# lly00412/MF-NeRF

Measured on AMD Instinct MI355X. Metric: training rays/sec + test PSNR, Synthetic-NeRF Lego 30k steps, higher is better.
Workload: dtype f16-mfma/f32; 1 GPU; Lego 800x800 training step, 8192 rays/batch/GPU, Hash L16 F2 T2^19, rgb 64x2; preset=lego, global_batch=8192, parallelism=dp1

## Files before the change

### mf-nerf_amd/csrc/vren_composite.hip

```cpp
#include "composite_sample.hpp"
#include "wave_ops.hpp"
#include "vren_launch.hpp"

using namespace mfn;
using namespace mfn_vren;

namespace {


__device__ __forceinline__ float t_chain(float a, float& T_run, float thr, int lane, int n_valid, int* stop) {
    constexpr int WAVE_SHR1 = 0x138;
    const float b = 1.0f - a;
    const float bs = __int_as_float(
        __builtin_amdgcn_update_dpp(__float_as_int(1.0f), __float_as_int(b), WAVE_SHR1, 0xF, 0xF, false));
    const int t0 = __float_as_int(T_run);
    float X = T_run;
    const int nv = __builtin_amdgcn_readfirstlane(n_valid);
    for (int k = 1; k < nv; ++k)
        X = __int_as_float(__builtin_amdgcn_update_dpp(t0, __float_as_int(X), WAVE_SHR1, 0xF, 0xF, false)) * bs;
    const float Ta = X * b;
    const uint64_t hit = __ballot(lane < n_valid && Ta <= thr);
    const int st = hit ? (int)__builtin_ctzll(hit) : 64;
    T_run = readlane_f(Ta, st < 64 ? st : n_valid - 1);
    *stop = st;
    return X;
}

__global__ __launch_bounds__(256) void composite_fw_wave_kernel(
    const float* __restrict__ sigmas, const float* __restrict__ rgbs, const float* __restrict__ deltas,
    const float* __restrict__ ts, const int64_t* __restrict__ rays_a, int64_t n_rays, float T_thr,
    int64_t* __restrict__ total_samples, float* __restrict__ opacity, float* __restrict__ depth,
    float* __restrict__ rgb, float* __restrict__ ws) {
    const int lane = threadIdx.x & 63;
    const int64_t n = ((int64_t)blockIdx.x * blockDim.x + threadIdx.x) >> 6;
    if (n >= n_rays) return;
    const int64_t ray = rays_a[3 * n], start = rays_a[3 * n + 1];
    const int N = (int)rays_a[3 * n + 2];
    float T = 1.0f, R = 0.f, G = 0.f, B = 0.f, D = 0.f, O = 0.f;
    int total = N;
    bool ended = false;
    for (int k0 = 0; k0 < N; k0 += 64) {
        const int nv = min(64, N - k0);
        const int64_t s = start + k0 + lane;
        const bool valid = lane < nv;
        float w = 0.0f;
        if (!ended) {
            const float a = valid ? 1.0f - fast_exp(-sigmas[s] * deltas[s]) : 0.0f;
            int stop;
            const float myT = t_chain(a, T, T_thr, lane, nv, &stop);
            if (valid && lane <= stop) {
                w = a * myT;
                R = fmaf(w, rgbs[3 * s], R); G = fmaf(w, rgbs[3 * s + 1], G); B = fmaf(w, rgbs[3 * s + 2], B);
                D = fmaf(w, ts[s], D);
                O += w;
            }
            if (stop < 64) { ended = true; total = k0 + stop; }
        }
        if (valid) ws[s] = w;
    }
    R = wave_sum(R); G = wave_sum(G); B = wave_sum(B); D = wave_sum(D); O = wave_sum(O);
    if (lane == 0) {
        opacity[ray] = O; depth[ray] = D;
        rgb[3 * ray] = R; rgb[3 * ray + 1] = G; rgb[3 * ray + 2] = B;
        total_samples[ray] = total;
    }
}

__global__ __launch_bounds__(256) void composite_bw_wave_kernel(
    const float* __restrict__ dL_dopacity, const float* __restrict__ dL_ddepth, const float* __restrict__ dL_drgb,
    const float* __restrict__ dL_dws, const float* __restrict__ sigmas, const float* __restrict__ rgbs,
    const float* __restrict__ ws, const float* __restrict__ deltas, const float* __restrict__ ts,
    const int64_t* __restrict__ rays_a, const float* __restrict__ opacity, const float* __restrict__ depth,
    const float* __restrict__ rgb, int64_t n_rays, float T_thr, float* __restrict__ dL_dsigmas,
    float* __restrict__ dL_drgbs) {
    const int lane = threadIdx.x & 63;
    const int64_t n = ((int64_t)blockIdx.x * blockDim.x + threadIdx.x) >> 6;
    if (n >= n_rays) return;
    const int64_t ray = rays_a[3 * n], start = rays_a[3 * n + 1];
    const int N = (int)rays_a[3 * n + 2];
    if (N <= 0) return;
    float wsum = 0.0f;
    for (int k0 = 0; k0 < N; k0 += 64) {
        const int64_t s = start + k0 + lane;
        if (k0 + lane < N) wsum += dL_dws[s] * ws[s];
    }
    wsum = wave_sum(wsum);
    const float Rt = rgb[3 * ray], Gt = rgb[3 * ray + 1], Bt = rgb[3 * ray + 2];
    const float O = opacity[ray], Dt = depth[ray];
    const float gr = dL_drgb[3 * ray], gg = dL_drgb[3 * ray + 1], gb = dL_drgb[3 * ray + 2];
    const float go = dL_dopacity[ray], gd = dL_ddepth[ray];
    float T = 1.0f, cr = 0.f, cg = 0.f, cb = 0.f, cd = 0.f, cs = 0.f;
    bool ended = false;
    for (int k0 = 0; k0 < N; k0 += 64) {
        const int nv = min(64, N - k0);
        const int64_t s = start + k0 + lane;
        const bool valid = lane < nv;
        float dsig = 0.0f, d0 = 0.0f, d1 = 0.0f, d2 = 0.0f;
        if (!ended) {
            float sg = 0.f, dl = 0.f, c0 = 0.f, c1 = 0.f, c2 = 0.f, tv = 0.f, dw = 0.f, wv = 0.f;
            if (valid) {
                sg = sigmas[s]; dl = deltas[s]; tv = ts[s]; dw = dL_dws[s]; wv = ws[s];
                c0 = rgbs[3 * s]; c1 = rgbs[3 * s + 1]; c2 = rgbs[3 * s + 2];
            }
            const float a = valid ? 1.0f - fast_exp(-sg * dl) : 0.0f;
            int stop;
            const float myT = t_chain(a, T, T_thr, lane, nv, &stop);
            const bool act = valid && lane <= stop;
            const float w = act ? a * myT : 0.0f;
            const float Tn = myT * (1.0f - a);
            const float pr = wave_incl_scan(w * c0) + cr, pg = wave_incl_scan(w * c1) + cg;
            const float pb = wave_incl_scan(w * c2) + cb, pd = wave_incl_scan(w * tv) + cd;
            const float ps = wave_incl_scan(act ? dw * wv : 0.0f) + cs;
            cr = readlane_f(pr, 63); cg = readlane_f(pg, 63); cb = readlane_f(pb, 63); cd = readlane_f(pd, 63);
            cs = readlane_f(ps, 63);
            if (act) {
                d0 = gr * w; d1 = gg * w; d2 = gb * w;
                float acc = gr * fmaf(c0, Tn, -(Rt - pr));
                acc = fmaf(gg, fmaf(c1, Tn, -(Gt - pg)), acc);
                acc = fmaf(gb, fmaf(c2, Tn, -(Bt - pb)), acc);
                acc = fmaf(go, 1 - O, acc);
                acc = fmaf(gd, fmaf(tv, Tn, -(Dt - pd)), acc);
                acc = fmaf(Tn, dw, acc);
                acc = acc - (wsum - ps);
                dsig = dl * acc;
            }
            if (stop < 64) ended = true;
        }
        if (valid) {
            dL_dsigmas[s] = dsig;
            dL_drgbs[3 * s] = d0; dL_drgbs[3 * s + 1] = d1; dL_drgbs[3 * s + 2] = d2;
        }
    }
}

struct BgUnused {};
template <bool DEV_BG> struct BgParam { using first = float; using rest = float; };
template <> struct BgParam<true> { using first = const float*; using rest = BgUnused; };
template <bool DEV_BG>
__device__ __forceinline__ void bg_fetch(typename BgParam<DEV_BG>::first a0, typename BgParam<DEV_BG>::rest a1,
                                         typename BgParam<DEV_BG>::rest a2, float& b0, float& b1, float& b2) {
    if constexpr (DEV_BG) { b0 = a0[0]; b1 = a0[1]; b2 = a0[2]; }
    else { b0 = a0; b1 = a1; b2 = a2; }
}

template <bool DEV_BG>
__global__ __launch_bounds__(256) void composite_fused_wave_kernel(
    const float* __restrict__ sigmas, const float* __restrict__ rgbs, const float* __restrict__ deltas,
    const float* __restrict__ ts, const int64_t* __restrict__ rays_a, int64_t n_rays, float T_thr,
    const float* __restrict__ target, int64_t n_mean, float lambda_o, typename BgParam<DEV_BG>::first bg0,
    typename BgParam<DEV_BG>::rest bg1, typename BgParam<DEV_BG>::rest bg2,
    int64_t* __restrict__ total_samples, float* __restrict__ opacity, float* __restrict__ depth,
    float* __restrict__ rgb, float* __restrict__ ws, float* __restrict__ dL_drgb, float* __restrict__ dL_dop,
    float* __restrict__ dL_dsigmas, float* __restrict__ dL_drgbs, float* __restrict__ loss_part) {
    __shared__ float lsum[4];
    const int lane = threadIdx.x & 63, wid = threadIdx.x >> 6;
    const int64_t n = ((int64_t)blockIdx.x * blockDim.x + threadIdx.x) >> 6;
    float l = 0.0f;
    if (n < n_rays) {
        const int64_t ray = rays_a[3 * n], start = rays_a[3 * n + 1];
        const int N = (int)rays_a[3 * n + 2];
        const float tg[3] = {target[3 * ray], target[3 * ray + 1], target[3 * ray + 2]};
        float b0, b1, b2;
        bg_fetch<DEV_BG>(bg0, bg1, bg2, b0, b1, b2);
        float T = 1.0f, R = 0.f, G = 0.f, B = 0.f, D = 0.f, O = 0.f;
        int total = N;
        bool ended = false;
        for (int k0 = 0; k0 < N; k0 += 64) {
            const int nv = min(64, N - k0);
            const int64_t s = start + k0 + lane;
            const bool valid = lane < nv;
            float w = 0.0f, tn = 0.0f;
            if (!ended) {
                float sg = 0.f, dl = 0.f, c0 = 0.f, c1 = 0.f, c2 = 0.f, tv = 0.f;
                if (valid) {
                    sg = sigmas[s]; dl = deltas[s]; tv = ts[s];
                    c0 = rgbs[3 * s]; c1 = rgbs[3 * s + 1]; c2 = rgbs[3 * s + 2];
                }
                const float a = valid ? 1.0f - fast_exp(-sg * dl) : 0.0f;
                int stop;
                const float myT = t_chain(a, T, T_thr, lane, nv, &stop);
                if (valid && lane <= stop) {
                    w = a * myT;
                    tn = myT * (1.0f - a);
                    R = fmaf(w, c0, R); G = fmaf(w, c1, G); B = fmaf(w, c2, B);
                    D = fmaf(w, tv, D);
                    O += w;
                }
                if (stop < 64) { ended = true; total = k0 + stop; }
            }
            if (valid) { ws[s] = w; dL_dsigmas[s] = tn; }
        }
        R = wave_sum(R); G = wave_sum(G); B = wave_sum(B); D = wave_sum(D); O = wave_sum(O);
        const float inv3n = 1.0f / (3.0f * (float)n_mean), invn = 1.0f / (float)n_mean;
        const float bg[3] = {b0, b1, b2}, col[3] = {R, G, B};
        float gcol[3], dop = 0.0f;
#pragma unroll
        for (int c = 0; c < 3; ++c) {
            const float e = col[c] + bg[c] * (1.0f - O) - tg[c];
            l += e * e * inv3n;
            gcol[c] = 2.0f * e * inv3n;
            dop -= bg[c] * gcol[c];
        }
        const float o = O + 1e-10f;
        l += lambda_o * (-o * logf(o)) * invn;
        const float go = dop + lambda_o * (-(logf(o) + 1.0f)) * invn;
        if (lane == 0) {
            opacity[ray] = O; depth[ray] = D;
            rgb[3 * ray] = R; rgb[3 * ray + 1] = G; rgb[3 * ray + 2] = B;
            total_samples[ray] = total;
            dL_drgb[3 * ray] = gcol[0]; dL_drgb[3 * ray + 1] = gcol[1]; dL_drgb[3 * ray + 2] = gcol[2];
            dL_dop[ray] = go;
        }
        const int last = ended ? total : N - 1;
        const float gr = gcol[0], gg = gcol[1], gb = gcol[2];
        float cr = 0.f, cg = 0.f, cb = 0.f;
        for (int k0 = 0; k0 < N; k0 += 64) {
            const int64_t s = start + k0 + lane;
            const bool valid = k0 + lane < N;
            const bool act = k0 + lane <= last;
            if (k0 > last) {
                if (valid) {
                    dL_dsigmas[s] = 0.0f;
                    dL_drgbs[3 * s] = 0.0f; dL_drgbs[3 * s + 1] = 0.0f; dL_drgbs[3 * s + 2] = 0.0f;
                }
                continue;
            }
            float w = 0.f, tn = 0.f, c0 = 0.f, c1 = 0.f, c2 = 0.f, dl = 0.f;
            if (act) {
                w = ws[s]; tn = dL_dsigmas[s]; dl = deltas[s];
                c0 = rgbs[3 * s]; c1 = rgbs[3 * s + 1]; c2 = rgbs[3 * s + 2];
            }
            const float pr = wave_incl_scan(w * c0) + cr, pg = wave_incl_scan(w * c1) + cg;
            const float pb = wave_incl_scan(w * c2) + cb;
            cr = readlane_f(pr, 63); cg = readlane_f(pg, 63); cb = readlane_f(pb, 63);
            float dsig = 0.0f, d0 = 0.0f, d1 = 0.0f, d2 = 0.0f;
            if (act) {
                d0 = gr * w; d1 = gg * w; d2 = gb * w;
                float acc = gr * fmaf(c0, tn, -(R - pr));
                acc = fmaf(gg, fmaf(c1, tn, -(G - pg)), acc);
                acc = fmaf(gb, fmaf(c2, tn, -(B - pb)), acc);
                acc = fmaf(go, 1 - O, acc);
                dsig = dl * acc;
            }
            if (valid) {
                dL_dsigmas[s] = dsig;
                dL_drgbs[3 * s] = d0; dL_drgbs[3 * s + 1] = d1; dL_drgbs[3 * s + 2] = d2;
            }
        }
    }
    if (lane == 0) lsum[wid] = l;
    __syncthreads();
    if (threadIdx.x == 0 && loss_part) loss_part[blockIdx.x] = (lsum[0] + lsum[1]) + (lsum[2] + lsum[3]);
}

__global__ void composite_test_kernel(const float* __restrict__ sigmas, const float* __restrict__ rgbs,
                                      const float* __restrict__ deltas, const float* __restrict__ ts,
                                      int64_t* __restrict__ alive, int64_t n_alive, int N_samples, float T_thr,
                                      const int32_t* __restrict__ n_eff, float* __restrict__ opacity,
                                      float* __restrict__ depth, float* __restrict__ rgb) {
    const int64_t n = (int64_t)blockIdx.x * blockDim.x + threadIdx.x;
    if (n >= n_alive) return;
    const int ne = n_eff[n];
    if (ne == 0) { alive[n] = -1; return; }
    const int64_t r = alive[n];
    RaySums S;
    S.O = opacity[r]; S.D = depth[r]; S.R = rgb[3 * r]; S.G = rgb[3 * r + 1]; S.B = rgb[3 * r + 2];
    S.T = 1 - S.O;
    for (int s = 0; s < ne; ++s) {
        const int64_t k = n * N_samples + s;
        const float sg = sigmas[k], dl = deltas[k];
        const float c0 = rgbs[3 * k], c1 = rgbs[3 * k + 1], c2 = rgbs[3 * k + 2];
        const float tv = ts[k];
        if (composite_sample(S, sg, dl, tv, c0, c1, c2, T_thr)) { alive[n] = -1; break; }
    }
    opacity[r] = S.O; depth[r] = S.D; rgb[3 * r] = S.R; rgb[3 * r + 1] = S.G; rgb[3 * r + 2] = S.B;
}

__global__ void distortion_fw_kernel(const float* __restrict__ ws, const float* __restrict__ deltas,
                                     const float* __restrict__ ts, const int64_t* __restrict__ rays_a,
                                     int64_t n_rays, float* __restrict__ loss, float* __restrict__ ws_incl,
                                     float* __restrict__ wts_incl) {
    const int64_t n = (int64_t)blockIdx.x * blockDim.x + threadIdx.x;
    if (n >= n_rays) return;
    const int64_t ray = rays_a[3 * n], start = rays_a[3 * n + 1];
    const int N = (int)rays_a[3 * n + 2];
    const float third = 1.0f / 3;
    float a = 0.f, b = 0.f, sum = 0.f;
    for (int k = 0; k < N; ++k) {
        const int64_t s = start + k;
        const float wx = a, wtx = b;
        a += ws[s]; b += ws[s] * ts[s];
        ws_incl[s] = a; wts_incl[s] = b;
        sum += 2 * (b * wx - a * wtx) + third * ws[s] * ws[s] * deltas[s];
    }
    loss[ray] = sum;
}

__global__ void distortion_bw_kernel(const float* __restrict__ dL_dloss, const float* __restrict__ ws_incl,
                                     const float* __restrict__ wts_incl, const float* __restrict__ ws,
                                     const float* __restrict__ deltas, const float* __restrict__ ts,
                                     const int64_t* __restrict__ rays_a, int64_t n_rays, float* __restrict__ dL_dws) {
    const int64_t n = (int64_t)blockIdx.x * blockDim.x + threadIdx.x;
    if (n >= n_rays) return;
    const int64_t ray = rays_a[3 * n], start = rays_a[3 * n + 1];
    const int N = (int)rays_a[3 * n + 2];
    if (N <= 0) return;
    const int64_t end = start + N - 1;
    const float ws_sum = ws_incl[end], wts_sum = wts_incl[end], g = dL_dloss[ray];
    for (int64_t s = start; s <= end; ++s) {
        const float first = (s == start) ? 0.0f : fmaf(ts[s], ws_incl[s - 1], -wts_incl[s - 1]);
        const float second = fmaf(-ts[s], ws_sum - ws_incl[s], wts_sum - wts_incl[s]);
        float v = g * 2 * (first + second);
        dL_dws[s] = fmaf(g * (float)2 / 3 * ws[s], deltas[s], v);
    }
}


template <bool DEV_BG>
__global__ void nerf_loss_kernel(const float* __restrict__ rgb, const float* __restrict__ opacity,
                                 const float* __restrict__ gt, int64_t n_rays, int64_t n_mean, float lambda_o,
                                 typename BgParam<DEV_BG>::first bg0, typename BgParam<DEV_BG>::rest bg1,
                                 typename BgParam<DEV_BG>::rest bg2, float* __restrict__ dL_drgb,
                                 float* __restrict__ dL_dop, float* __restrict__ loss_sum) {
    const int64_t r = (int64_t)blockIdx.x * blockDim.x + threadIdx.x;
    float l = 0.0f;
    if (r < n_rays) {
        const float op = opacity[r];
        const float inv3n = 1.0f / (3.0f * (float)n_mean), invn = 1.0f / (float)n_mean;
        float b0, b1, b2;
        bg_fetch<DEV_BG>(bg0, bg1, bg2, b0, b1, b2);
        const float bg[3] = {b0, b1, b2};
        float dop = 0.0f;
#pragma unroll
        for (int c = 0; c < 3; ++c) {
            const float e = rgb[3 * r + c] + bg[c] * (1.0f - op) - gt[3 * r + c];
            l += e * e * inv3n;
            const float g = 2.0f * e * inv3n;
            dL_drgb[3 * r + c] = g;
            dop -= bg[c] * g;
        }
        const float o = op + 1e-10f;
        l += lambda_o * (-o * logf(o)) * invn;
        dL_dop[r] = dop + lambda_o * (-(logf(o) + 1.0f)) * invn;
    }
    for (int off = 32; off > 0; off >>= 1) l += __shfl_down(l, off, 64);
    if ((threadIdx.x & 63) == 0 && loss_sum) atomicAdd(loss_sum, l);
}

template <bool DEV_BG>
int composite_train_fused_launch(const char* what, const float* sigmas, const float* rgbs, const float* deltas,
                                 const float* ts, const int64_t* rays_a, int64_t n_rays, int64_t n_samples,
                                 float T_threshold, const float* target, int64_t n_mean, float lambda_opacity,
                                 typename BgParam<DEV_BG>::first bg0, typename BgParam<DEV_BG>::rest bg1,
                                 typename BgParam<DEV_BG>::rest bg2, int64_t* total_samples, float* opacity,
                                 float* depth, float* rgb, float* ws, float* dL_drgb, float* dL_dopacity,
                                 float* dL_dsigmas, float* dL_drgbs, float* loss_partials, mfnerf_stream_t stream) {
    if (n_rays < 0 || n_samples < 0 || n_mean < 0 || (n_mean > 0 && n_mean < n_rays)) {
        mfn_set_error("%s: bad sizes", what); return MFN_ERR_INVALID;
    }
    if (n_mean == 0) n_mean = n_rays;
    if (n_rays == 0) return MFN_OK;
    if (!rays_a || !target || !total_samples || !opacity || !depth || !rgb || !dL_drgb || !dL_dopacity ||
        (n_samples > 0 && (!sigmas || !rgbs || !deltas || !ts || !ws || !dL_dsigmas || !dL_drgbs))) {
        mfn_set_error("%s: null pointer", what); return MFN_ERR_INVALID;
    }
    hipLaunchKernelGGL(composite_fused_wave_kernel<DEV_BG>, dim3(blocks_for(n_rays, 4)), dim3(256), 0, stream, sigmas,
                       rgbs, deltas, ts, rays_a, n_rays, T_threshold, target, n_mean, lambda_opacity, bg0, bg1, bg2,
                       total_samples, opacity, depth, rgb, ws, dL_drgb, dL_dopacity, dL_dsigmas, dL_drgbs,
                       loss_partials);
    return mfn_check_launch(what);
}

template <bool DEV_BG>
int nerf_loss_launch(const char* what, const float* rgb, const float* opacity, const float* target, int64_t n_rays,
                     int64_t n_mean, float lambda_opacity, typename BgParam<DEV_BG>::first bg0,
                     typename BgParam<DEV_BG>::rest bg1, typename BgParam<DEV_BG>::rest bg2, float* dL_drgb,
                     float* dL_dopacity, float* loss_sum, mfnerf_stream_t stream) {
    if (n_rays < 0 || n_mean < 0 || (n_mean > 0 && n_mean < n_rays)) {
        mfn_set_error("%s: bad size", what); return MFN_ERR_INVALID;
    }
    if (n_mean == 0) n_mean = n_rays;
    if (n_rays == 0) return MFN_OK;
    if (!rgb || !opacity || !target || !dL_drgb || !dL_dopacity) {
        mfn_set_error("%s: null pointer", what); return MFN_ERR_INVALID;
    }
    hipLaunchKernelGGL(nerf_loss_kernel<DEV_BG>, dim3(blocks_for(n_rays, 256)), dim3(256), 0, stream, rgb, opacity,
                       target, n_rays, n_mean, lambda_opacity, bg0, bg1, bg2, dL_drgb, dL_dopacity, loss_sum);
    return mfn_check_launch(what);
}

}

extern "C" {

int mfnerf_composite_train_fw(const float* sigmas, const float* rgbs, const float* deltas, const float* ts,
                              const int64_t* rays_a, int64_t n_rays, int64_t n_samples, float T_threshold,
                              int64_t* total_samples, float* opacity, float* depth, float* rgb, float* ws,
                              mfnerf_stream_t stream) {
    if (n_rays < 0 || n_samples < 0) { mfn_set_error("composite_train_fw: bad sizes"); return MFN_ERR_INVALID; }
    if (n_rays == 0) return MFN_OK;
    if (!rays_a || !total_samples || !opacity || !depth || !rgb ||
        (n_samples > 0 && (!sigmas || !rgbs || !deltas || !ts || !ws))) {
        mfn_set_error("composite_train_fw: null pointer"); return MFN_ERR_INVALID;
    }
    hipLaunchKernelGGL(composite_fw_wave_kernel, dim3(blocks_for(n_rays, 4)), dim3(256), 0, stream, sigmas, rgbs, deltas,
                       ts, rays_a, n_rays, T_threshold, total_samples, opacity, depth, rgb, ws);
    return mfn_check_launch("composite_train_fw");
}

int mfnerf_composite_train_bw(const float* dL_dopacity, const float* dL_ddepth, const float* dL_drgb,
                              const float* dL_dws, const float* sigmas, const float* rgbs, const float* ws,
                              const float* deltas, const float* ts, const int64_t* rays_a, const float* opacity,
                              const float* depth, const float* rgb, int64_t n_rays, int64_t n_samples,
                              float T_threshold, float* dL_dsigmas, float* dL_drgbs, mfnerf_stream_t stream) {
    if (n_rays < 0 || n_samples < 0) { mfn_set_error("composite_train_bw: bad sizes"); return MFN_ERR_INVALID; }
    if (n_rays == 0) return MFN_OK;
    if (!dL_dopacity || !dL_ddepth || !dL_drgb || !rays_a || !opacity || !depth || !rgb ||
        (n_samples > 0 && (!dL_dws || !sigmas || !rgbs || !ws || !deltas || !ts || !dL_dsigmas || !dL_drgbs))) {
        mfn_set_error("composite_train_bw: null pointer"); return MFN_ERR_INVALID;
    }
    hipLaunchKernelGGL(composite_bw_wave_kernel, dim3(blocks_for(n_rays, 4)), dim3(256), 0, stream,
                       dL_dopacity, dL_ddepth, dL_drgb, dL_dws, sigmas, rgbs, ws, deltas, ts, rays_a, opacity,
                       depth, rgb, n_rays, T_threshold, dL_dsigmas, dL_drgbs);
    return mfn_check_launch("composite_train_bw");
}

int mfnerf_composite_train_fused(const float* sigmas, const float* rgbs, const float* deltas, const float* ts,
                                 const int64_t* rays_a, int64_t n_rays, int64_t n_samples, float T_threshold,
                                 const float* target, int64_t n_mean, float lambda_opacity, float bg_r, float bg_g,
                                 float bg_b, int64_t* total_samples, float* opacity, float* depth, float* rgb,
                                 float* ws, float* dL_drgb, float* dL_dopacity, float* dL_dsigmas, float* dL_drgbs,
                                 float* loss_partials, mfnerf_stream_t stream) {
    return composite_train_fused_launch<false>("composite_train_fused", sigmas, rgbs, deltas, ts, rays_a, n_rays,
                                               n_samples, T_threshold, target, n_mean, lambda_opacity, bg_r, bg_g, bg_b,
                                               total_samples, opacity, depth, rgb, ws, dL_drgb, dL_dopacity,
                                               dL_dsigmas, dL_drgbs, loss_partials, stream);
}

int mfnerf_composite_train_fused_bg(const float* sigmas, const float* rgbs, const float* deltas, const float* ts,
                                    const int64_t* rays_a, int64_t n_rays, int64_t n_samples, float T_threshold,
                                    const float* target, int64_t n_mean, float lambda_opacity, const float* bg,
                                    int64_t* total_samples, float* opacity, float* depth, float* rgb, float* ws,
                                    float* dL_drgb, float* dL_dopacity, float* dL_dsigmas, float* dL_drgbs,
                                    float* loss_partials, mfnerf_stream_t stream) {
    if (!bg) { mfn_set_error("composite_train_fused_bg: null bg"); return MFN_ERR_INVALID; }
    return composite_train_fused_launch<true>("composite_train_fused_bg", sigmas, rgbs, deltas, ts, rays_a, n_rays,
                                              n_samples, T_threshold, target, n_mean, lambda_opacity, bg, BgUnused{},
                                              BgUnused{}, total_samples, opacity, depth, rgb, ws, dL_drgb, dL_dopacity,
                                              dL_dsigmas, dL_drgbs, loss_partials, stream);
}

int mfnerf_composite_test_fw(const float* sigmas, const float* rgbs, const float* deltas, const float* ts,
                             int64_t* alive_indices, int64_t n_alive, int N_samples, float T_threshold,
                             const int32_t* n_eff, float* opacity, float* depth, float* rgb,
                             mfnerf_stream_t stream) {
    if (n_alive < 0 || N_samples < 0) { mfn_set_error("composite_test_fw: bad sizes"); return MFN_ERR_INVALID; }
    if (n_alive == 0) return MFN_OK;
    if (!alive_indices || !n_eff || !opacity || !depth || !rgb ||
        (N_samples > 0 && (!sigmas || !rgbs || !deltas || !ts))) {
        mfn_set_error("composite_test_fw: null pointer"); return MFN_ERR_INVALID;
    }
    hipLaunchKernelGGL(composite_test_kernel, dim3(blocks_for(n_alive, RAY_BLOCK)), dim3(RAY_BLOCK), 0, stream,
                       sigmas, rgbs, deltas, ts, alive_indices, n_alive, N_samples, T_threshold, n_eff, opacity,
                       depth, rgb);
    return mfn_check_launch("composite_test_fw");
}

int mfnerf_distortion_loss_fw(const float* ws, const float* deltas, const float* ts, const int64_t* rays_a,
                              int64_t n_rays, int64_t n_samples, float* loss, float* ws_incl, float* wts_incl,
                              mfnerf_stream_t stream) {
    if (n_rays < 0 || n_samples < 0) { mfn_set_error("distortion_loss_fw: bad sizes"); return MFN_ERR_INVALID; }
    if (n_rays == 0) return MFN_OK;
    if (!rays_a || !loss || (n_samples > 0 && (!ws || !deltas || !ts || !ws_incl || !wts_incl))) {
        mfn_set_error("distortion_loss_fw: null pointer"); return MFN_ERR_INVALID;
    }
    mfn_zero_async(loss, n_rays * sizeof(float), stream);
    hipLaunchKernelGGL(distortion_fw_kernel, dim3(blocks_for(n_rays, RAY_BLOCK)), dim3(RAY_BLOCK), 0, stream, ws,
                       deltas, ts, rays_a, n_rays, loss, ws_incl, wts_incl);
    return mfn_check_launch("distortion_loss_fw");
}

int mfnerf_distortion_loss_bw(const float* dL_dloss, const float* ws_incl, const float* wts_incl,
                              const float* ws, const float* deltas, const float* ts, const int64_t* rays_a,
                              int64_t n_rays, int64_t n_samples, float* dL_dws, mfnerf_stream_t stream) {
    if (n_rays < 0 || n_samples < 0) { mfn_set_error("distortion_loss_bw: bad sizes"); return MFN_ERR_INVALID; }
    if (n_rays == 0) return MFN_OK;
    if (!dL_dloss || !rays_a || (n_samples > 0 && (!ws_incl || !wts_incl || !ws || !deltas || !ts || !dL_dws))) {
        mfn_set_error("distortion_loss_bw: null pointer"); return MFN_ERR_INVALID;
    }
    if (n_samples > 0) mfn_zero_async(dL_dws, n_samples * sizeof(float), stream);
    hipLaunchKernelGGL(distortion_bw_kernel, dim3(blocks_for(n_rays, RAY_BLOCK)), dim3(RAY_BLOCK), 0, stream,
                       dL_dloss, ws_incl, wts_incl, ws, deltas, ts, rays_a, n_rays, dL_dws);
    return mfn_check_launch("distortion_loss_bw");
}

int mfnerf_nerf_loss(const float* rgb, const float* opacity, const float* target, int64_t n_rays, int64_t n_mean,
                     float lambda_opacity, float bg_r, float bg_g, float bg_b, float* dL_drgb, float* dL_dopacity,
                     float* loss_sum, mfnerf_stream_t stream) {
    return nerf_loss_launch<false>("nerf_loss", rgb, opacity, target, n_rays, n_mean, lambda_opacity, bg_r, bg_g, bg_b,
                                   dL_drgb, dL_dopacity, loss_sum, stream);
}

int mfnerf_nerf_loss_bg(const float* rgb, const float* opacity, const float* target, int64_t n_rays, int64_t n_mean,
                        float lambda_opacity, const float* bg, float* dL_drgb, float* dL_dopacity, float* loss_sum,
                        mfnerf_stream_t stream) {
    if (!bg) { mfn_set_error("nerf_loss_bg: null bg"); return MFN_ERR_INVALID; }
    return nerf_loss_launch<true>("nerf_loss_bg", rgb, opacity, target, n_rays, n_mean, lambda_opacity, bg, BgUnused{},
                                  BgUnused{}, dL_drgb, dL_dopacity, loss_sum, stream);
}

}
```

Baseline: 17.89 million rays/s.

## Prefetch next sample chunk and hand-schedule DPP transmittance chain in composite kernels

Forward, backward and fused composite kernels now load the next 64-sample chunk and compute its alpha while the current chunk's transmittance scan runs, so global-load latency overlaps the serial DPP chain. The transmittance chain is rewritten as inline-asm v_mul_f32_dpp with an unroll of 8, and the fused kernel keeps the first chunk's data in registers instead of writing and re-reading it. The wsum pre-pass is unrolled four ways. The cost is more register pressure from the prefetched chunk. The chain also rounds its iteration count up to a multiple of 8, which can add wasted steps for short rays.

```diff
diff --git a/mf-nerf_amd/csrc/vren_composite.hip b/mf-nerf_amd/csrc/vren_composite.hip
--- a/mf-nerf_amd/csrc/vren_composite.hip
+++ b/mf-nerf_amd/csrc/vren_composite.hip
@@ -7,17 +7,21 @@
 
 namespace {
 
+
+constexpr int CHAIN_UNROLL = 8;
 
 __device__ __forceinline__ float t_chain(float a, float& T_run, float thr, int lane, int n_valid, int* stop) {
     constexpr int WAVE_SHR1 = 0x138;
     const float b = 1.0f - a;
     const float bs = __int_as_float(
         __builtin_amdgcn_update_dpp(__float_as_int(1.0f), __float_as_int(b), WAVE_SHR1, 0xF, 0xF, false));
-    const int t0 = __float_as_int(T_run);
     float X = T_run;
     const int nv = __builtin_amdgcn_readfirstlane(n_valid);
-    for (int k = 1; k < nv; ++k)
-        X = __int_as_float(__builtin_amdgcn_update_dpp(t0, __float_as_int(X), WAVE_SHR1, 0xF, 0xF, false)) * bs;
+    for (int k = 1; k < nv; k += CHAIN_UNROLL) {
+#pragma unroll
+        for (int u = 0; u < CHAIN_UNROLL; ++u)
+            asm("s_nop 1\n\tv_mul_f32_dpp %0, %0, %1 wave_shr:1 row_mask:0xf bank_mask:0xf" : "+v"(X) : "v"(bs));
+    }
     const float Ta = X * b;
     const uint64_t hit = __ballot(lane < n_valid && Ta <= thr);
     const int st = hit ? (int)__builtin_ctzll(hit) : 64;
@@ -26,43 +30,75 @@
     return X;
 }
 
+
+__device__ __forceinline__ int64_t wave_ray() {
+    return (int64_t)blockIdx.x * 4 + __builtin_amdgcn_readfirstlane(threadIdx.x >> 6);
+}
+
+__device__ __forceinline__ void pin(float& x) { asm volatile("" : "+v"(x) : : "memory"); }
+
+struct ChunkIn { float sg, dl, tv, c0, c1, c2; };
+
+__device__ __forceinline__ ChunkIn load_chunk(const float* __restrict__ sigmas, const float* __restrict__ rgbs,
+                                              const float* __restrict__ deltas, const float* __restrict__ ts,
+                                              int64_t s, bool on) {
+    ChunkIn c = {0.f, 0.f, 0.f, 0.f, 0.f, 0.f};
+    if (on) {
+        const float *pc = rgbs + 3 * s, *pt = ts + s, *ps = sigmas + s, *pd = deltas + s;
+        c.c0 = pc[0]; c.c1 = pc[1]; c.c2 = pc[2]; c.tv = *pt; c.sg = *ps; c.dl = *pd;
+    }
+    return c;
+}
+__device__ __forceinline__ float chunk_alpha(const ChunkIn& c, bool on) {
+    return on ? 1.0f - fast_exp(-c.sg * c.dl) : 0.0f;
+}
+
+struct RayFw { float T, R, G, B, D, O; int total; bool ended; };
+__device__ __forceinline__ void fw_chunk(RayFw& f, float a, const ChunkIn& c, float thr, int lane, int nv, int k0,
+                                         float& w, float& tn) {
+    int stop;
+    const float myT = t_chain(a, f.T, thr, lane, nv, &stop);
+    if (lane < nv && lane <= stop) {
+        w = a * myT;
+        tn = myT * (1.0f - a);
+        f.R = fmaf(w, c.c0, f.R); f.G = fmaf(w, c.c1, f.G); f.B = fmaf(w, c.c2, f.B);
+        f.D = fmaf(w, c.tv, f.D);
+        f.O += w;
+    }
+    if (stop < 64) { f.ended = true; f.total = k0 + stop; }
+}
+
 __global__ __launch_bounds__(256) void composite_fw_wave_kernel(
     const float* __restrict__ sigmas, const float* __restrict__ rgbs, const float* __restrict__ deltas,
     const float* __restrict__ ts, const int64_t* __restrict__ rays_a, int64_t n_rays, float T_thr,
     int64_t* __restrict__ total_samples, float* __restrict__ opacity, float* __restrict__ depth,
     float* __restrict__ rgb, float* __restrict__ ws) {
     const int lane = threadIdx.x & 63;
-    const int64_t n = ((int64_t)blockIdx.x * blockDim.x + threadIdx.x) >> 6;
+    const int64_t n = wave_ray();
     if (n >= n_rays) return;
     const int64_t ray = rays_a[3 * n], start = rays_a[3 * n + 1];
     const int N = (int)rays_a[3 * n + 2];
-    float T = 1.0f, R = 0.f, G = 0.f, B = 0.f, D = 0.f, O = 0.f;
-    int total = N;
-    bool ended = false;
+    RayFw f = {1.0f, 0.f, 0.f, 0.f, 0.f, 0.f, N, false};
+    ChunkIn cur = load_chunk(sigmas, rgbs, deltas, ts, start + lane, lane < N);
+    float a = chunk_alpha(cur, lane < N);
+    pin(a);
     for (int k0 = 0; k0 < N; k0 += 64) {
         const int nv = min(64, N - k0);
         const int64_t s = start + k0 + lane;
-        const bool valid = lane < nv;
-        float w = 0.0f;
-        if (!ended) {
-            const float a = valid ? 1.0f - fast_exp(-sigmas[s] * deltas[s]) : 0.0f;
-            int stop;
-            const float myT = t_chain(a, T, T_thr, lane, nv, &stop);
-            if (valid && lane <= stop) {
-                w = a * myT;
-                R = fmaf(w, rgbs[3 * s], R); G = fmaf(w, rgbs[3 * s + 1], G); B = fmaf(w, rgbs[3 * s + 2], B);
-                D = fmaf(w, ts[s], D);
-                O += w;
-            }
-            if (stop < 64) { ended = true; total = k0 + stop; }
-        }
-        if (valid) ws[s] = w;
-    }
-    R = wave_sum(R); G = wave_sum(G); B = wave_sum(B); D = wave_sum(D); O = wave_sum(O);
+        const bool more = k0 + 64 + lane < N;
+        const ChunkIn nxt = load_chunk(sigmas, rgbs, deltas, ts, s + 64, more && !f.ended);
+        float w = 0.0f, tn = 0.0f;
+        if (!f.ended) fw_chunk(f, a, cur, T_thr, lane, nv, k0, w, tn);
+        a = chunk_alpha(nxt, more);
+        pin(a);
+        if (lane < nv) ws[s] = w;
+        cur = nxt;
+    }
+    const float R = wave_sum(f.R), G = wave_sum(f.G), B = wave_sum(f.B), D = wave_sum(f.D), O = wave_sum(f.O);
     if (lane == 0) {
         opacity[ray] = O; depth[ray] = D;
         rgb[3 * ray] = R; rgb[3 * ray + 1] = G; rgb[3 * ray + 2] = B;
-        total_samples[ray] = total;
+        total_samples[ray] = f.total;
     }
 }
 
@@ -74,15 +110,22 @@
     const float* __restrict__ rgb, int64_t n_rays, float T_thr, float* __restrict__ dL_dsigmas,
     float* __restrict__ dL_drgbs) {
     const int lane = threadIdx.x & 63;
-    const int64_t n = ((int64_t)blockIdx.x * blockDim.x + threadIdx.x) >> 6;
+    const int64_t n = wave_ray();
     if (n >= n_rays) return;
     const int64_t ray = rays_a[3 * n], start = rays_a[3 * n + 1];
     const int N = (int)rays_a[3 * n + 2];
     if (N <= 0) return;
     float wsum = 0.0f;
-    for (int k0 = 0; k0 < N; k0 += 64) {
-        const int64_t s = start + k0 + lane;
-        if (k0 + lane < N) wsum += dL_dws[s] * ws[s];
+    for (int k0 = 0; k0 < N; k0 += 256) {
+        float p[4];
+#pragma unroll
+        for (int u = 0; u < 4; ++u) {
+            const int k = k0 + 64 * u + lane;
+            p[u] = k < N ? dL_dws[start + k] * ws[start + k] : 0.0f;
+        }
+#pragma unroll
+        for (int u = 0; u < 4; ++u)
+            if (k0 + 64 * u + lane < N) wsum += p[u];
     }
     wsum = wave_sum(wsum);
     const float Rt = rgb[3 * ray], Gt = rgb[3 * ray + 1], Bt = rgb[3 * ray + 2];
@@ -91,18 +134,22 @@
     const float go = dL_dopacity[ray], gd = dL_ddepth[ray];
     float T = 1.0f, cr = 0.f, cg = 0.f, cb = 0.f, cd = 0.f, cs = 0.f;
     bool ended = false;
+    ChunkIn cur = load_chunk(sigmas, rgbs, deltas, ts, start + lane, lane < N);
+    float dw = 0.f, wv = 0.f;
+    if (lane < N) { dw = dL_dws[start + lane]; wv = ws[start + lane]; }
+    float a = chunk_alpha(cur, lane < N);
+    pin(a);
     for (int k0 = 0; k0 < N; k0 += 64) {
         const int nv = min(64, N - k0);
         const int64_t s = start + k0 + lane;
         const bool valid = lane < nv;
+        const bool more = k0 + 64 + lane < N && !ended;
+        float ndw = 0.f, nwv = 0.f;
+        if (more) { ndw = dL_dws[s + 64]; nwv = ws[s + 64]; }
+        const ChunkIn nxt = load_chunk(sigmas, rgbs, deltas, ts, s + 64, more);
         float dsig = 0.0f, d0 = 0.0f, d1 = 0.0f, d2 = 0.0f;
         if (!ended) {
-            float sg = 0.f, dl = 0.f, c0 = 0.f, c1 = 0.f, c2 = 0.f, tv = 0.f, dw = 0.f, wv = 0.f;
-            if (valid) {
-                sg = sigmas[s]; dl = deltas[s]; tv = ts[s]; dw = dL_dws[s]; wv = ws[s];
-                c0 = rgbs[3 * s]; c1 = rgbs[3 * s + 1]; c2 = rgbs[3 * s + 2];
-            }
-            const float a = valid ? 1.0f - fast_exp(-sg * dl) : 0.0f;
+            const float dl = cur.dl, c0 = cur.c0, c1 = cur.c1, c2 = cur.c2, tv = cur.tv;
             int stop;
             const float myT = t_chain(a, T, T_thr, lane, nv, &stop);
             const bool act = valid && lane <= stop;
@@ -126,10 +173,13 @@
             }
             if (stop < 64) ended = true;
         }
+        a = chunk_alpha(nxt, k0 + 64 + lane < N);
+        pin(a);
         if (valid) {
             dL_dsigmas[s] = dsig;
             dL_drgbs[3 * s] = d0; dL_drgbs[3 * s + 1] = d1; dL_drgbs[3 * s + 2] = d2;
         }
+        cur = nxt; dw = ndw; wv = nwv;
     }
 }
 
@@ -141,6 +191,33 @@
                                          typename BgParam<DEV_BG>::rest a2, float& b0, float& b1, float& b2) {
     if constexpr (DEV_BG) { b0 = a0[0]; b1 = a0[1]; b2 = a0[2]; }
     else { b0 = a0; b1 = a1; b2 = a2; }
+}
+
+
+struct FusedBwIn { float w, tn, dl, c0, c1, c2; };
+
+struct FusedBwRay { float gr, gg, gb, go, R, G, B, O, cr, cg, cb; };
+
+__device__ __forceinline__ void fused_bw_chunk(FusedBwRay& r, const FusedBwIn& v, FusedBwIn& nxt, bool act, bool valid,
+                                               int64_t s, float* __restrict__ dL_dsigmas,
+                                               float* __restrict__ dL_drgbs) {
+    const float pr = wave_incl_scan(v.w * v.c0) + r.cr, pg = wave_incl_scan(v.w * v.c1) + r.cg;
+    const float pb = wave_incl_scan(v.w * v.c2) + r.cb;
+    r.cr = readlane_f(pr, 63); r.cg = readlane_f(pg, 63); r.cb = readlane_f(pb, 63);
+    float dsig = 0.0f, d0 = 0.0f, d1 = 0.0f, d2 = 0.0f;
+    if (act) {
+        d0 = r.gr * v.w; d1 = r.gg * v.w; d2 = r.gb * v.w;
+        float acc = r.gr * fmaf(v.c0, v.tn, -(r.R - pr));
+        acc = fmaf(r.gg, fmaf(v.c1, v.tn, -(r.G - pg)), acc);
+        acc = fmaf(r.gb, fmaf(v.c2, v.tn, -(r.B - pb)), acc);
+        acc = fmaf(r.go, 1 - r.O, acc);
+        dsig = v.dl * acc;
+    }
+    pin(nxt.w); pin(nxt.tn); pin(nxt.dl); pin(nxt.c0); pin(nxt.c1); pin(nxt.c2);
+    if (valid) {
+        dL_dsigmas[s] = dsig;
+        dL_drgbs[3 * s] = d0; dL_drgbs[3 * s + 1] = d1; dL_drgbs[3 * s + 2] = d2;
+    }
 }
 
 template <bool DEV_BG>
@@ -154,7 +231,7 @@
     float* __restrict__ dL_dsigmas, float* __restrict__ dL_drgbs, float* __restrict__ loss_part) {
     __shared__ float lsum[4];
     const int lane = threadIdx.x & 63, wid = threadIdx.x >> 6;
-    const int64_t n = ((int64_t)blockIdx.x * blockDim.x + threadIdx.x) >> 6;
+    const int64_t n = wave_ray();
     float l = 0.0f;
     if (n < n_rays) {
         const int64_t ray = rays_a[3 * n], start = rays_a[3 * n + 1];
@@ -162,35 +239,40 @@
         const float tg[3] = {target[3 * ray], target[3 * ray + 1], target[3 * ray + 2]};
         float b0, b1, b2;
         bg_fetch<DEV_BG>(bg0, bg1, bg2, b0, b1, b2);
-        float T = 1.0f, R = 0.f, G = 0.f, B = 0.f, D = 0.f, O = 0.f;
-        int total = N;
-        bool ended = false;
+        RayFw f = {1.0f, 0.f, 0.f, 0.f, 0.f, 0.f, N, false};
+        ChunkIn cur = load_chunk(sigmas, rgbs, deltas, ts, start + lane, lane < N);
+        float a = chunk_alpha(cur, lane < N);
+        pin(a);
+        FusedBwIn first = {0.f, 0.f, 0.f, 0.f, 0.f, 0.f};
         for (int k0 = 0; k0 < N; k0 += 64) {
             const int nv = min(64, N - k0);
             const int64_t s = start + k0 + lane;
-            const bool valid = lane < nv;
+            const bool more = k0 + 64 + lane < N;
+            const ChunkIn nxt = load_chunk(sigmas, rgbs, deltas, ts, s + 64, more && !f.ended);
             float w = 0.0f, tn = 0.0f;
-            if (!ended) {
-                float sg = 0.f, dl = 0.f, c0 = 0.f, c1 = 0.f, c2 = 0.f, tv = 0.f;
-                if (valid) {
-                    sg = sigmas[s]; dl = deltas[s]; tv = ts[s];
-                    c0 = rgbs[3 * s]; c1 = rgbs[3 * s + 1]; c2 = rgbs[3 * s + 2];
-                }
-                const float a = valid ? 1.0f - fast_exp(-sg * dl) : 0.0f;
-                int stop;
-                const float myT = t_chain(a, T, T_thr, lane, nv, &stop);
-                if (valid && lane <= stop) {
-                    w = a * myT;
-                    tn = myT * (1.0f - a);
-                    R = fmaf(w, c0, R); G = fmaf(w, c1, G); B = fmaf(w, c2, B);
-                    D = fmaf(w, tv, D);
-                    O += w;
-                }
-                if (stop < 64) { ended = true; total = k0 + stop; }
+            if (!f.ended) fw_chunk(f, a, cur, T_thr, lane, nv, k0, w, tn);
+            a = chunk_alpha(nxt, more);
+            pin(a);
+            if (k0 == 0) {
+                first = {w, tn, cur.dl, cur.c0, cur.c1, cur.c2};
+                if (lane < nv) ws[s] = w;
+            } else if (lane < nv) {
+                ws[s] = w; dL_dsigmas[s] = tn;
             }
-            if (valid) { ws[s] = w; dL_dsigmas[s] = tn; }
-        }
-        R = wave_sum(R); G = wave_sum(G); B = wave_sum(B); D = wave_sum(D); O = wave_sum(O);
+            cur = nxt;
+        }
+        const int last = f.ended ? f.total : N - 1;
+        const auto load_bw = [&](int k0) {
+            FusedBwIn v = {0.f, 0.f, 0.f, 0.f, 0.f, 0.f};
+            if (k0 + lane <= last) {
+                const int64_t s = start + k0 + lane;
+                const float *pw = ws + s, *pt = dL_dsigmas + s, *pd = deltas + s, *pc = rgbs + 3 * s;
+                v.w = *pw; v.tn = *pt; v.dl = *pd; v.c0 = pc[0]; v.c1 = pc[1]; v.c2 = pc[2];
+            }
+            return v;
+        };
+        FusedBwIn bcur = load_bw(64);
+        const float R = wave_sum(f.R), G = wave_sum(f.G), B = wave_sum(f.B), D = wave_sum(f.D), O = wave_sum(f.O);
         const float inv3n = 1.0f / (3.0f * (float)n_mean), invn = 1.0f / (float)n_mean;
         const float bg[3] = {b0, b1, b2}, col[3] = {R, G, B};
         float gcol[3], dop = 0.0f;
@@ -207,44 +289,27 @@
         if (lane == 0) {
             opacity[ray] = O; depth[ray] = D;
             rgb[3 * ray] = R; rgb[3 * ray + 1] = G; rgb[3 * ray + 2] = B;
-            total_samples[ray] = total;
+            total_samples[ray] = f.total;
             dL_drgb[3 * ray] = gcol[0]; dL_drgb[3 * ray + 1] = gcol[1]; dL_drgb[3 * ray + 2] = gcol[2];
             dL_dop[ray] = go;
         }
-        const int last = ended ? total : N - 1;
-        const float gr = gcol[0], gg = gcol[1], gb = gcol[2];
-        float cr = 0.f, cg = 0.f, cb = 0.f;
-        for (int k0 = 0; k0 < N; k0 += 64) {
+        FusedBwRay r = {gcol[0], gcol[1], gcol[2], go, R, G, B, O, 0.f, 0.f, 0.f};
+        {
+            const bool act = lane <= last;
+            if (!act) first.dl = first.c0 = first.c1 = first.c2 = 0.0f;
+            fused_bw_chunk(r, first, bcur, act, lane < N, start + lane, dL_dsigmas, dL_drgbs);
+        }
+        int k0 = 64;
+        for (; k0 <= last; k0 += 64) {
+            FusedBwIn bnxt = load_bw(k0 + 64);
+            fused_bw_chunk(r, bcur, bnxt, k0 + lane <= last, k0 + lane < N, start + k0 + lane, dL_dsigmas, dL_drgbs);
+            bcur = bnxt;
+        }
+        for (; k0 < N; k0 += 64) {
             const int64_t s = start + k0 + lane;
-            const bool valid = k0 + lane < N;
-            const bool act = k0 + lane <= last;
-            if (k0 > last) {
-                if (valid) {
-                    dL_dsigmas[s] = 0.0f;
-                    dL_drgbs[3 * s] = 0.0f; dL_drgbs[3 * s + 1] = 0.0f; dL_drgbs[3 * s + 2] = 0.0f;
-                }
-                continue;
-            }
-            float w = 0.f, tn = 0.f, c0 = 0.f, c1 = 0.f, c2 = 0.f, dl = 0.f;
-            if (act) {
-                w = ws[s]; tn = dL_dsigmas[s]; dl = deltas[s];
-                c0 = rgbs[3 * s]; c1 = rgbs[3 * s + 1]; c2 = rgbs[3 * s + 2];
-            }
-            const float pr = wave_incl_scan(w * c0) + cr, pg = wave_incl_scan(w * c1) + cg;
-            const float pb = wave_incl_scan(w * c2) + cb;
-            cr = readlane_f(pr, 63); cg = readlane_f(pg, 63); cb = readlane_f(pb, 63);
-            float dsig = 0.0f, d0 = 0.0f, d1 = 0.0f, d2 = 0.0f;
-            if (act) {
-                d0 = gr * w; d1 = gg * w; d2 = gb * w;
-                float acc = gr * fmaf(c0, tn, -(R - pr));
-                acc = fmaf(gg, fmaf(c1, tn, -(G - pg)), acc);
-                acc = fmaf(gb, fmaf(c2, tn, -(B - pb)), acc);
-                acc = fmaf(go, 1 - O, acc);
-                dsig = dl * acc;
-            }
-            if (valid) {
-                dL_dsigmas[s] = dsig;
-                dL_drgbs[3 * s] = d0; dL_drgbs[3 * s + 1] = d1; dL_drgbs[3 * s + 2] = d2;
+            if (k0 + lane < N) {
+                dL_dsigmas[s] = 0.0f;
+                dL_drgbs[3 * s] = 0.0f; dL_drgbs[3 * s + 1] = 0.0f; dL_drgbs[3 * s + 2] = 0.0f;
             }
         }
     }
```

New measurement: 17.88 million rays/s. About the same (-0.0%).
